# aluo7/ViT-SOM

Hardware: AMD Instinct MI355X
Metric: images/sec/node ViT-SOM 40x40 CIFAR-10 bs512 (training step: fwd+bwd+all-reduce+AdamW) (higher is better)
Workload: dtype f32 (Linear GEMMs on bf16 MFMA: forward from an exact 3xbf16 operand split, six products; weight / input gradients from a 2xbf16 split, three products, rel. error 4e-6)

## Files before the change

vit_som_amd/csrc/bmu_x3.hip:

```cpp
#include "gemm_x6.h"
#include "adamw.h"

#include <type_traits>

namespace vsom {

constexpr float BMU_WINDOW = 2.0e-4f;

struct BmuP {
    const float* X; long ldx; const float* W;
    int B, K, L;
    int ktiles_per_split;
    float* slab; long slab_stride;
    float* xsq; float* wsq;
    unsigned x_bytes, w_bytes;
};

template <int WM, int WN, int WAVES_M, int WAVES_N>
__global__ __launch_bounds__(WAVES_M * WAVES_N * 64) void bmu_x3_kernel(const BmuP g) {
    constexpr int BM = WAVES_M * WM * 32, BN = WAVES_N * WN * 32, NT = WAVES_M * WAVES_N * 64, RPP = NT / 8;
    constexpr int PA = BM * X6_RS, PB = BN * X6_RS;
    __shared__ __attribute__((aligned(16))) char lds[2 * (PA + PB)];
    char* As = lds; char* Bs = lds + 2 * PA;
    const int t = threadIdx.x, lane = t & 63, wave = t >> 6;
// ... 26 lines not shown
    const bool want_x = tn == 0, want_w = tm == 0;
    float ssa[BM / RPP], ssb[BN / RPP];
#pragma unroll
    for (int p = 0; p < BM / RPP; ++p) ssa[p] = 0.f;
#pragma unroll
    for (int p = 0; p < BN / RPP; ++p) ssb[p] = 0.f;

    auto gload = [&](int kt) {
        load_kc_fast<BM, NT>(sa, rsA, oa, kt << 5, g.L, t);
        load_kc_fast<BN, NT>(sb, rsB, ob, kt << 5, g.L, t);
    };
    auto lstore = [&](int) {
#pragma unroll
        for (int p = 0; p < BM / RPP; ++p) {
            const f32x4 v = sa.v[p];
            if (want_x) ssa[p] += (v[0] * v[0] + v[1] * v[1]) + (v[2] * v[2] + v[3] * v[3]);
            uint2 p1, p2;
            x3_split(v, p1, p2);
            char* dst = As + x6_piece_off(p * RPP + (t >> 3), t & 7);
            *reinterpret_cast<uint2*>(dst) = p1;
            *reinterpret_cast<uint2*>(dst + PA) = p2;
        }
#pragma unroll
        for (int p = 0; p < BN / RPP; ++p) {
            const f32x4 v = sb.v[p];
            if (want_w) ssb[p] += (v[0] * v[0] + v[1] * v[1]) + (v[2] * v[2] + v[3] * v[3]);
            uint2 p1, p2;
            x3_split(v, p1, p2);
            char* dst = Bs + x6_piece_off(p * RPP + (t >> 3), t & 7);
            *reinterpret_cast<uint2*>(dst) = p1;
            *reinterpret_cast<uint2*>(dst + PB) = p2;
        }
    };
    auto mfma_tile = [&](int) {
#pragma unroll
        for (int ks = 0; ks < 2; ++ks) {
            bf16x8 a[WM][2], b[WN][2];
#pragma unroll
            for (int i = 0; i < WM; ++i)
#pragma unroll
                for (int pl = 0; pl < 2; ++pl)
                    a[i][pl] = *reinterpret_cast<const bf16x8*>(As + pl * PA + x6_chunk_off(wm0 + i * 32 + r, 2 * ks + h));
#pragma unroll
            for (int j = 0; j < WN; ++j)
#pragma unroll
                for (int pl = 0; pl < 2; ++pl)
                    b[j][pl] = *reinterpret_cast<const bf16x8*>(Bs + pl * PB + x6_chunk_off(wn0 + j * 32 + r, 2 * ks + h));
#pragma unroll
            for (int i = 0; i < WM; ++i)
#pragma unroll
                for (int j = 0; j < WN; ++j) x6_products<2>(acc[i][j], a[i], b[j]);
        }
    };
    X6_KLOOP(1, 2 * (PA + PB), kt_begin, kt_end, gload, lstore, mfma_tile);

    if (want_x) {
#pragma unroll
        for (int p = 0; p < BM / RPP; ++p) {
            float v = ssa[p];
            v += __shfl_xor(v, 1, 64); v += __shfl_xor(v, 2, 64); v += __shfl_xor(v, 4, 64);
            const int m = bm0 + p * RPP + (t >> 3);
            if ((t & 7) == 0 && m < g.B) g.xsq[(long)z * g.B + m] = v;
        }
    }
    if (want_w) {
#pragma unroll
        for (int p = 0; p < BN / RPP; ++p) {
            float v = ssb[p];
            v += __shfl_xor(v, 1, 64); v += __shfl_xor(v, 2, 64); v += __shfl_xor(v, 4, 64);
            const int n = bn0 + p * RPP + (t >> 3);
            if ((t & 7) == 0 && n < g.K) g.wsq[(long)z * g.K + n] = v;
        }
    }
    float* sl = g.slab + (long)z * g.slab_stride;
#pragma unroll
    for (int i = 0; i < WM; ++i)
#pragma unroll
        for (int j = 0; j < WN; ++j) {
            const int n = bn0 + wn0 + j * 32 + r;
            if (n >= g.K) continue;
            const int mb = bm0 + wm0 + i * 32 + 4 * h;
#pragma unroll
            for (int v = 0; v < 16; ++v) {
                const int m = mb + (v & 3) + 8 * (v >> 2);
                if (m < g.B) sl[(long)m * g.K + n] = acc[i][j][v];
            }
        }
}

__global__ __launch_bounds__(256) void bmu_norms_kernel(const float* __restrict__ xsq, const float* __restrict__ wsq, int nz,
                                                        int B, int K, float* __restrict__ inv_nx, float* __restrict__ inv_nw) {
    const int i = blockIdx.x * 256 + threadIdx.x;
    if (i >= B + K) return;
    const bool isx = i < B;
    const float* p = isx ? xsq + i : wsq + (i - B);
    const int n = isx ? B : K;
    float s = 0.f;
    for (int z = 0; z < nz; ++z) s += p[(long)z * n];
    const float inv = 1.0f / fmaxf(sqrtf(s), 1e-12f);
    if (isx) inv_nx[i] = inv; else inv_nw[i - B] = inv;
}

__global__ __launch_bounds__(512) void bmu_norms_wide_kernel(const float* __restrict__ xsq, const float* __restrict__ wsq, int nz,
                                                             int B, int K, float* __restrict__ inv_nx, float* __restrict__ inv_nw) {
    __shared__ float part[8][64];
    const int lane = threadIdx.x & 63, w = threadIdx.x >> 6;
    const int i = blockIdx.x * 64 + lane;
// ... 577 lines not shown
```

vit_som_amd/csrc/gemm_f32.h:

```cpp
#pragma once
#include "common.h"

namespace vsom {

enum Epi : int {
    EPI_NONE = 0,
    EPI_BIAS = 1,
    EPI_BIAS_GELU = 2,
    EPI_BIAS_RES = 3,
    EPI_ROWAXPY = 4,
    EPI_GELU_BWD = 5,
    EPI_SLAB = 6,
    EPI_BIAS_RELU = 7,
    EPI_LN_BWD = 8,
};

struct GemmP {
    const float* A; const float* B; float* C;
    long lda, ldb, ldc;
    int M, N, K;
    int ktiles_per_split;
    int a_seg, a_stride, a_off;
    int c_seg, c_stride, c_off;
    const float* bias;
// ... 81 lines not shown
                v[0] = src[0];
                if (k + 1 < K) v[1] = src[1];
                if (k + 2 < K) v[2] = src[2];
                if (k + 3 < K) v[3] = src[3];
            }
        }
        s.v[p] = v;
    }
}
template <int ROWS>
__device__ __forceinline__ void store_kc(const StageRegs<ROWS>& s, float* lds, int t) {
#pragma unroll
    for (int p = 0; p < ROWS / 32; ++p)
        *reinterpret_cast<f32x4*>(lds + (p * 32 + (t >> 3)) * 36 + ((t & 7) << 2)) = s.v[p];
}
template <int COLS>
__device__ __forceinline__ void load_ks(StageRegs<COLS>& s, const float* __restrict__ base, long ld,
                                        int col0, int ncols, int k0, int K, int vec, int t, int seg,
                                        int stride, int off) {
    constexpr int TPR = COLS / 4;
    constexpr int KPP = 256 / TPR;
#pragma unroll
    for (int p = 0; p < COLS / 32; ++p) {
        const int k = k0 + p * KPP + t / TPR;
        const int col = col0 + ((t % TPR) << 2);
        f32x4 v = {0.f, 0.f, 0.f, 0.f};
        if (k < K && col < ncols) {
            const long row = seg ? (long)(k / seg) * stride + off + (k % seg) : (long)k;
            const float* src = base + row * ld + col;
            if (vec && col + 3 < ncols) {
                v = *reinterpret_cast<const f32x4*>(src);
            } else {
                v[0] = src[0];
                if (col + 1 < ncols) v[1] = src[1];
                if (col + 2 < ncols) v[2] = src[2];
                if (col + 3 < ncols) v[3] = src[3];
            }
        }
        s.v[p] = v;
    }
}
template <int COLS>
__device__ __forceinline__ void store_ks(const StageRegs<COLS>& s, float* lds, int t) {
    constexpr int TPR = COLS / 4;
    constexpr int KPP = 256 / TPR;
#pragma unroll
    for (int p = 0; p < COLS / 32; ++p)
        *reinterpret_cast<f32x4*>(lds + (p * KPP + t / TPR) * (COLS + 4) + ((t % TPR) << 2)) = s.v[p];
}

template <int WM, int WN, int EPI>
__device__ __forceinline__ void gemm_epilogue(const GemmP& g, const f32x16 (&acc)[WM][WN], int m0, int n0, int r, int h, int z) {
    const bool rowmap = (EPI == EPI_BIAS_RES) && g.c_seg != 0;
#pragma unroll
    for (int i = 0; i < WM; ++i) {
#pragma unroll
        for (int j = 0; j < WN; ++j) {
            const int n = n0 + j * 32 + r;
            if (n >= g.N) continue;
            const int mb = m0 + i * 32 + 4 * h;
            float bn = 0.f;
            if constexpr (EPI == EPI_BIAS || EPI == EPI_BIAS_GELU || EPI == EPI_BIAS_RELU || EPI == EPI_BIAS_RES) bn = g.bias ? g.bias[n] : 0.f;
            const bool plain_rows = (m0 + i * 32 + 31 < g.M) && !rowmap &&
                                    !((EPI == EPI_BIAS_RES) && !(g.r_mod >= g.M && g.r_off == 0));
            if (plain_rows) {
                float* d = (EPI == EPI_SLAB) ? g.slab + (long)z * g.slab_stride + (long)mb * g.N + n : g.C + (long)mb * g.ldc + n;
                const long dstep = (EPI == EPI_SLAB) ? (long)g.N : g.ldc;
                const float* rp = nullptr;
                float* d2 = nullptr;
                if constexpr (EPI == EPI_ROWAXPY || EPI == EPI_GELU_BWD || EPI == EPI_BIAS_RES) rp = g.R + (long)mb * g.ldr + n;
                if constexpr (EPI == EPI_BIAS_GELU || EPI == EPI_BIAS_RELU) d2 = g.C2 + (long)mb * g.ldc2 + n;
                const float* rs = nullptr;
                if constexpr (EPI == EPI_ROWAXPY) rs = g.rowscale + mb;
                constexpr bool READS_R = (EPI == EPI_ROWAXPY || EPI == EPI_GELU_BWD || EPI == EPI_BIAS_RES);
                constexpr bool MAY_ACC = (EPI == EPI_NONE || EPI == EPI_ROWAXPY || EPI == EPI_GELU_BWD);
                float rv[16], dv[16];
                if constexpr (READS_R) {
                    const float* q = rp;
#pragma unroll
                    for (int v = 0; v < 16; ++v) { rv[v] = *q; q += (((v & 3) == 3) ? 5 : 1) * g.ldr; }
                }
                float sv[16];
                if constexpr (EPI == EPI_ROWAXPY) {
#pragma unroll
                    for (int v = 0; v < 16; ++v) sv[v] = rs[(v & 3) + 8 * (v >> 2)];
                }
                const bool accum = MAY_ACC && g.accumulate;
                if (accum) {
                    const float* q = d;
#pragma unroll
                    for (int v = 0; v < 16; ++v) { dv[v] = *q; q += (((v & 3) == 3) ? 5 : 1) * dstep; }
                }
#pragma unroll
                for (int v = 0; v < 16; ++v) {
                    const float a = acc[i][j][v];
                    if constexpr (EPI == EPI_SLAB) {
                        *d = a;
                    } else if constexpr (EPI == EPI_NONE) {
                        float val = g.alpha * a;
                        if (accum) val += dv[v];
                        *d = val;
                    } else if constexpr (EPI == EPI_BIAS) {
                        *d = a + bn;
                    } else if constexpr (EPI == EPI_BIAS_GELU) {
                        float act, grad;
                        gelu_erf_both(a + bn, act, grad);
                        *d = grad;
                        *d2 = act;
                    } else if constexpr (EPI == EPI_BIAS_RELU) {
                        const float pre = a + bn;
                        *d = pre > 0.f ? 1.0f : 0.f;
                        *d2 = fmaxf(pre, 0.f);
                    } else if constexpr (EPI == EPI_BIAS_RES) {
                        *d = a + bn + rv[v];
                    } else if constexpr (EPI == EPI_ROWAXPY) {
                        float val = a + sv[v] * rv[v];
                        if (accum) val += dv[v];
                        *d = val;
                    } else if constexpr (EPI == EPI_GELU_BWD) {
                        float val = a * rv[v];
                        if (accum) val += dv[v];
                        *d = val;
                    }
                    const long adv = ((v & 3) == 3) ? 5 : 1;
                    d += adv * dstep;
                    if constexpr (EPI == EPI_BIAS_GELU || EPI == EPI_BIAS_RELU) d2 += adv * g.ldc2;
                }
                continue;
            }
            if constexpr (EPI == EPI_SLAB) {
                float* dst = g.slab + (long)z * g.slab_stride + (long)mb * g.N + n;
#pragma unroll
                for (int v = 0; v < 16; ++v) {
                    const int dm = (v & 3) + 8 * (v >> 2);
                    if (mb + dm < g.M) dst[(long)dm * g.N] = acc[i][j][v];
                }
            } else if (rowmap) {
#pragma unroll
                for (int v = 0; v < 16; ++v) {
                    const int m = mb + (v & 3) + 8 * (v >> 2);
                    if (m >= g.M) continue;
                    const long orow = (long)(m / g.c_seg) * g.c_stride + g.c_off + (m % g.c_seg);
                    const long rr = (long)(m % g.r_mod) + g.r_off;
                    g.C[orow * g.ldc + n] = acc[i][j][v] + bn + g.R[rr * g.ldr + n];
                }
            } else {
                float* dst = g.C + (long)mb * g.ldc + n;
                const float* rsrc = nullptr;
                float* dst2 = nullptr;
                if constexpr (EPI == EPI_ROWAXPY || EPI == EPI_GELU_BWD) rsrc = g.R + (long)mb * g.ldr + n;
                if constexpr (EPI == EPI_BIAS_GELU || EPI == EPI_BIAS_RELU) dst2 = g.C2 + (long)mb * g.ldc2 + n;
                const bool plain_res = (EPI == EPI_BIAS_RES) && g.r_mod >= g.M && g.r_off == 0;
                if constexpr (EPI == EPI_BIAS_RES) rsrc = g.R + (long)mb * g.ldr + n;
#pragma unroll
                for (int v = 0; v < 16; ++v) {
                    const int dm = (v & 3) + 8 * (v >> 2);
                    const int m = mb + dm;
                    if (m >= g.M) continue;
                    const float a = acc[i][j][v];
                    float* d = dst + (long)dm * g.ldc;
                    if constexpr (EPI == EPI_NONE) {
                        float val = g.alpha * a;
                        if (g.accumulate) val += *d;
                        *d = val;
                    } else if constexpr (EPI == EPI_BIAS) {
                        *d = a + bn;
                    } else if constexpr (EPI == EPI_BIAS_GELU) {
                        float act, grad;
                        gelu_erf_both(a + bn, act, grad);
                        *d = grad;
                        dst2[(long)dm * g.ldc2] = act;
                    } else if constexpr (EPI == EPI_BIAS_RELU) {
                        const float pre = a + bn;
// ... 131 lines not shown
                    for (int j = 0; j < WN; ++j)
                        acc[i][j] = __builtin_amdgcn_mfma_f32_32x32x2f32(a[i][s], b[j][s], acc[i][j], 0, 0, 0);
        }
    };
    for (int kt = kt_begin; kt + 1 < kt_end; ++kt) {
        gload(kt + 1);
        __builtin_amdgcn_sched_barrier(0);
        mfma_tile();
        __syncthreads();
        lstore();
        __syncthreads();
    }
    if (kt_begin < kt_end) mfma_tile();

    if constexpr (EPI == EPI_SLAB) {
        if (want_colsum && t < BM && bm0 + t < g.M) g.slab_bias[(long)z * g.slab_bias_stride + bm0 + t] = colsum;
    }
    gemm_epilogue<WM, WN, EPI>(g, acc, bm0 + wm0, bn0 + wn0, r, h, z);
}

enum GemmEngine : int { GEMM_ENGINE_F32 = 0, GEMM_ENGINE_X6 = 1 };
struct GemmPlan {
    int engine;
    int tile_m;
    int planes;
    bool fast;
    int splits;
    int ktiles_per_split;
    int tiles;
    int grid;
};
GemmPlan gemm_plan(bool a_kc, bool b_kc, int epi, int M, int N, int K, bool fast, int mode, int products, int splits);
int gemm_mode();
int launch_gemm(bool a_kc, bool b_kc, int epi, GemmP g, int splits, hipStream_t stream);
int linear_bwd_weight_impl(const float* dY, long lddy, const float* X, long ldx, float* dW, float* db, int M, int N,
                           int K, int a_seg, int a_stride, int a_off, void* ws, size_t ws_bytes,
                           hipStream_t stream);
template <int WAVES, int VEC>
__device__ __forceinline__ void reduce_slabs_body(f32x4 (*sh)[64], int bx, const float* __restrict__ slabs, long stride,
                                                  int nslabs, float* __restrict__ out1, long n1,
                                                  float* __restrict__ out2, long off2, long n2,
                                                  int nb1, int vec) {
    const int lane = threadIdx.x & 63, wave = threadIdx.x >> 6;
    const bool seg2 = bx >= nb1;
    const long col = ((long)(seg2 ? bx - nb1 : bx) * 64 + lane) * VEC;
    const long n = seg2 ? n2 : n1;
    const float* src = slabs + (seg2 ? off2 : 0) + col;
    f32x4 acc[4];
#pragma unroll
    for (int u = 0; u < 4; ++u) acc[u] = f32x4{0.f, 0.f, 0.f, 0.f};
    if (col < n) {
        if (VEC == 4 && vec && col + 3 < n) {
            int s = wave;
            for (; s + 3 * WAVES < nslabs; s += 4 * WAVES) {
#pragma unroll
                for (int u = 0; u < 4; ++u) acc[u] += *reinterpret_cast<const f32x4*>(src + (long)(s + u * WAVES) * stride);
            }
            for (; s < nslabs; s += WAVES) acc[0] += *reinterpret_cast<const f32x4*>(src + (long)s * stride);
        } else if (VEC == 1) {
            int s = wave;
            for (; s + 3 * WAVES < nslabs; s += 4 * WAVES) {
#pragma unroll
                for (int u = 0; u < 4; ++u) acc[u][0] += src[(long)(s + u * WAVES) * stride];
            }
            for (; s < nslabs; s += WAVES) acc[0][0] += src[(long)s * stride];
        } else {
            for (int s = wave; s < nslabs; s += WAVES)
#pragma unroll
                for (int e = 0; e < 4; ++e)
                    if (col + e < n) acc[0][e] += src[(long)s * stride + e];
        }
    }
    sh[wave][lane] = (acc[0] + acc[1]) + (acc[2] + acc[3]);
    __syncthreads();
    if (wave == 0 && col < n) {
        f32x4 t = sh[0][lane];
#pragma unroll
        for (int w = 1; w < WAVES; ++w) t += sh[w][lane];
        float* dst = (seg2 ? out2 : out1) + col;
        if (VEC == 1) {
            dst[0] = t[0];
        } else if (col + 3 < n && (reinterpret_cast<uintptr_t>(dst) & 15u) == 0) {
            *reinterpret_cast<f32x4*>(dst) = t;
        } else {
#pragma unroll
            for (int e = 0; e < 4; ++e)
                if (col + e < n) dst[e] = t[e];
        }
    }
}

int reduce_slabs_internal(const float* slabs, long stride, int nslabs, float* out, long n, hipStream_t stream);
int reduce_slabs2_internal(const float* slabs, long stride, int nslabs, float* out1, long n1, float* out2, long off2,
                           long n2, hipStream_t stream);
int sum_partials(const float* part, int n, float* out, hipStream_t stream);
int choose_splits(int tiles, int ktiles, int max_splits, bool prefer_xcd_multiple = false);
int bmu_splits(int B, int K, int L);
int attn_bwd_threads(int N);
int attn_bwd_plan_now(int N, int hd);
int gemm_grad_products();

}
```

vit_som_amd/csrc/gemm_x6.h:

```cpp
#pragma once
#include "gemm_f32.h"
#include "layernorm_bwd.h"

namespace vsom {

typedef __attribute__((ext_vector_type(8))) __bf16 bf16x8;
typedef unsigned v4u32 __attribute__((ext_vector_type(4)));

__device__ __forceinline__ unsigned x6_bits(float x) { return __builtin_bit_cast(unsigned, x); }
__device__ __forceinline__ float x6_float(unsigned x) { return __builtin_bit_cast(float, x); }

__device__ __forceinline__ void x6_split(f32x4 v, uint2& p1, uint2& p2, uint2& p3) {
    const unsigned HI = 0xffff0000u, SEL = 0x07060302u;
    float r[4], s[4];
#pragma unroll
    for (int e = 0; e < 4; ++e) {
        r[e] = v[e] - x6_float(x6_bits(v[e]) & HI);
        s[e] = r[e] - x6_float(x6_bits(r[e]) & HI);
    }
    p1.x = __builtin_amdgcn_perm(x6_bits(v[1]), x6_bits(v[0]), SEL); p1.y = __builtin_amdgcn_perm(x6_bits(v[3]), x6_bits(v[2]), SEL);
    p2.x = __builtin_amdgcn_perm(x6_bits(r[1]), x6_bits(r[0]), SEL); p2.y = __builtin_amdgcn_perm(x6_bits(r[3]), x6_bits(r[2]), SEL);
    p3.x = __builtin_amdgcn_perm(x6_bits(s[1]), x6_bits(s[0]), SEL); p3.y = __builtin_amdgcn_perm(x6_bits(s[3]), x6_bits(s[2]), SEL);
}

// ... 14 lines not shown

template <int ROWS, int NPL = 3, int NT = 256>
__device__ __forceinline__ void x6_store(const StageRegs<ROWS, NT>& s, char* planes, int t) {
    constexpr int PL = ROWS * X6_RS;
#pragma unroll
    for (int p = 0; p < ROWS * 8 / NT; ++p) {
        uint2 p1, p2, p3;
        if constexpr (NPL == 3) x6_split(s.v[p], p1, p2, p3); else x3_split(s.v[p], p1, p2);
        char* dst = planes + x6_piece_off(p * (NT / 8) + (t >> 3), t & 7);
        *reinterpret_cast<uint2*>(dst) = p1;
        *reinterpret_cast<uint2*>(dst + PL) = p2;
        if constexpr (NPL == 3) *reinterpret_cast<uint2*>(dst + 2 * PL) = p3;
    }
}

struct X6Blk { f32x4 v[4]; };
__device__ __forceinline__ void x6_load_ks(X6Blk& b, __amdgpu_buffer_rsrc_t rsrc, unsigned colbytes, unsigned ld4, int k0,
                                           int K, int kg, int seg, int stride, int off0) {
#pragma unroll
    for (int i = 0; i < 4; ++i) {
        const int k = k0 + 4 * kg + i;
        const unsigned row = seg ? (unsigned)((k / seg) * stride + off0 + (k % seg)) : (unsigned)k;
        b.v[i] = bload4(rsrc, (k < K && colbytes != OOB) ? row * ld4 + colbytes : OOB);
    }
}
template <int NPL = 3>
__device__ __forceinline__ void x6_store_ks(const X6Blk& b, char* planes, int plane_bytes, int mq, int kg) {
#pragma unroll
    for (int e = 0; e < 4; ++e) {
        const f32x4 col = {b.v[0][e], b.v[1][e], b.v[2][e], b.v[3][e]};
        uint2 p1, p2, p3;
        if constexpr (NPL == 3) x6_split(col, p1, p2, p3); else x3_split(col, p1, p2);
        char* dst = planes + x6_piece_off(4 * mq + e, kg);
        *reinterpret_cast<uint2*>(dst) = p1;
        *reinterpret_cast<uint2*>(dst + plane_bytes) = p2;
        if constexpr (NPL == 3) *reinterpret_cast<uint2*>(dst + 2 * plane_bytes) = p3;
    }
}

template <int NPL>
__device__ __forceinline__ void x6_products(f32x16& acc, const bf16x8 (&a)[NPL], const bf16x8 (&b)[NPL]) {
    f32x16 c = acc;
    if constexpr (NPL == 3) {
        c = __builtin_amdgcn_mfma_f32_32x32x16_bf16(a[2], b[0], c, 0, 0, 0);
        c = __builtin_amdgcn_mfma_f32_32x32x16_bf16(a[0], b[2], c, 0, 0, 0);
        c = __builtin_amdgcn_mfma_f32_32x32x16_bf16(a[1], b[1], c, 0, 0, 0);
    }
    c = __builtin_amdgcn_mfma_f32_32x32x16_bf16(a[1], b[0], c, 0, 0, 0);
    c = __builtin_amdgcn_mfma_f32_32x32x16_bf16(a[0], b[1], c, 0, 0, 0);
    c = __builtin_amdgcn_mfma_f32_32x32x16_bf16(a[0], b[0], c, 0, 0, 0);
    acc = c;
}

#define X6_KLOOP(STAGES, ST, kt_begin, kt_end, gload, lstore, mfma_tile)                                                    \
    do {                                                                                                                    \
        static_assert((STAGES) == 1 || (STAGES) == 2, "one or two LDS stages");                                            \
        if constexpr ((STAGES) == 1) {                                                                                      \
            if ((kt_begin) < (kt_end)) {                                                                                    \
                gload(kt_begin);                                                                                            \
                lstore(0);                                                                                                  \
            }                                                                                                               \
            __syncthreads();                                                                                                \
            for (int kt_ = (kt_begin); kt_ + 1 < (kt_end); ++kt_) {                                                         \
                gload(kt_ + 1);                                                                                             \
                __builtin_amdgcn_sched_barrier(0);                                                                          \
                mfma_tile(0);                                                                                               \
                __builtin_amdgcn_sched_barrier(0);                                                                          \
                __syncthreads();                                                                                            \
                lstore(0);                                                                                                  \
                __syncthreads();                                                                                            \
            }                                                                                                               \
            if ((kt_begin) < (kt_end)) mfma_tile(0);                                                                        \
        } else {                                                                                                            \
            if ((kt_begin) < (kt_end)) {                                                                                    \
                gload(kt_begin);                                                                                            \
                lstore(0);                                                                                                  \
                if ((kt_begin) + 1 < (kt_end)) gload((kt_begin) + 1);                                                       \
            }                                                                                                               \
            __syncthreads();                                                                                                \
            int so_ = 0;                                                                                                    \
            for (int kt_ = (kt_begin); kt_ + 1 < (kt_end); ++kt_) {                                                         \
                lstore((ST) - so_);                                                                                         \
                gload(kt_ + 2 < (kt_end) ? kt_ + 2 : kt_ + 1);                                                              \
                __builtin_amdgcn_sched_barrier(0);                                                                          \
                mfma_tile(so_);                                                                                             \
                __builtin_amdgcn_sched_barrier(0);                                                                          \
                __syncthreads();                                                                                            \
                so_ = (ST) - so_;                                                                                           \
            }                                                                                                               \
            if ((kt_begin) < (kt_end)) mfma_tile(so_);                                                                      \
        }                                                                                                                   \
    } while (0)

template <int WN, int WAVES_M, int WAVES_N, int LDS_BYTES>
__device__ __forceinline__ void x6_ln_bwd_epilogue(const GemmP& g, const f32x16 (&acc)[1][WN], char* lds, int bm0, int wm0,
                                                   int wn0, int r, int h, int tile, int t) {
    constexpr int BN = WAVES_N * WN * 32;
    constexpr int cols = BN;
    constexpr int NCH = (BN + 63) / 64;
    constexpr int LROW = BN + 8;
    constexpr int PROWS = WAVES_M * 8;
    constexpr int ITER = PROWS / 16;
    static_assert(PROWS % 16 == 0 && PROWS * LROW * 4 <= LDS_BYTES && 16 * 2 * BN * 4 <= LDS_BYTES, "LN epilogue does not fit");
    float* st = reinterpret_cast<float*>(lds);
    const int sub = t & 15, rg = t >> 4;
    const float inv_n = 1.0f / (float)cols;
    const unsigned rbytes = (unsigned)g.M * cols * 4u;
    const __amdgpu_buffer_rsrc_t rsX = __builtin_amdgcn_make_buffer_rsrc(const_cast<float*>(g.ln_x), 0, (int)rbytes, 0x00020000);
    const __amdgpu_buffer_rsrc_t rsR = __builtin_amdgcn_make_buffer_rsrc(const_cast<float*>(g.ln_resid), 0, (int)rbytes, 0x00020000);
    const __amdgpu_buffer_rsrc_t rsD = __builtin_amdgcn_make_buffer_rsrc(g.C, 0, (int)rbytes, 0x00020000);
    const __amdgpu_buffer_rsrc_t rsM = __builtin_amdgcn_make_buffer_rsrc(const_cast<float*>(g.ln_mean), 0, g.M * 4, 0x00020000);
    const __amdgpu_buffer_rsrc_t rsS = __builtin_amdgcn_make_buffer_rsrc(const_cast<float*>(g.ln_rstd), 0, g.M * 4, 0x00020000);
    const bool has_resid = g.ln_resid != nullptr;
    f32x4 gam[NCH], dg[NCH], db[NCH];
    bool cv[NCH];
#pragma unroll
    for (int j = 0; j < NCH; ++j) {
        cv[j] = 4 * (sub + 16 * j) < cols;
        gam[j] = cv[j] ? reinterpret_cast<const f32x4*>(g.ln_gamma)[sub + 16 * j] : f32x4{0.f, 0.f, 0.f, 0.f};
        dg[j] = f32x4{0.f, 0.f, 0.f, 0.f};
        db[j] = f32x4{0.f, 0.f, 0.f, 0.f};
    }
    const int wr = wm0 >> 5;
#pragma unroll
    for (int q = 0; q < 4; ++q) {
        bool ok[ITER];
        unsigned off[ITER][NCH];
        float mu[ITER], rs[ITER];
        f32x4 xv[ITER][NCH], rr[ITER][NCH];
#pragma unroll
        for (int i = 0; i < ITER; ++i) {
            const int lr = 16 * i + rg;
            const int row = bm0 + (lr >> 3) * 32 + 8 * q + (lr & 7);
            ok[i] = row < g.M;
#pragma unroll
            for (int j = 0; j < NCH; ++j)
                off[i][j] = (ok[i] && cv[j]) ? (unsigned)row * (cols * 4u) + 16u * (sub + 16 * j) : OOB;
            const unsigned roff = ok[i] ? (unsigned)row * 4u : OOB;
            mu[i] = __builtin_bit_cast(float, __builtin_amdgcn_raw_buffer_load_b32(rsM, (int)roff, 0, 0));
            rs[i] = __builtin_bit_cast(float, __builtin_amdgcn_raw_buffer_load_b32(rsS, (int)roff, 0, 0));
#pragma unroll
            for (int j = 0; j < NCH; ++j) {
                xv[i][j] = bload4(rsX, off[i][j]);
                rr[i][j] = has_resid ? bload4(rsR, off[i][j]) : f32x4{0.f, 0.f, 0.f, 0.f};
            }
        }
        __syncthreads();
#pragma unroll
        for (int j = 0; j < WN; ++j)
#pragma unroll
            for (int e = 0; e < 4; ++e) st[(wr * 8 + e + 4 * h) * LROW + wn0 + j * 32 + r] = acc[0][j][4 * q + e];
        __syncthreads();
#pragma unroll
        for (int i = 0; i < ITER; ++i) {
            const int lr = 16 * i + rg;
            f32x4 d[NCH], o[NCH];
#pragma unroll
            for (int j = 0; j < NCH; ++j) {
                d[j] = (cv[j] && ok[i]) ? *reinterpret_cast<const f32x4*>(st + lr * LROW + 4 * (sub + 16 * j)) : f32x4{0.f, 0.f, 0.f, 0.f};
                if (!cv[j]) xv[i][j] = f32x4{mu[i], mu[i], mu[i], mu[i]};
            }
            ln_bwd_row<NCH>(d, xv[i], mu[i], rs[i], gam, inv_n, o, dg, db);
#pragma unroll
            for (int j = 0; j < NCH; ++j) {
                if (has_resid) ln_bwd_add_resid(o[j], rr[i][j]);
                __builtin_amdgcn_raw_buffer_store_b128(__builtin_bit_cast(v4u32, o[j]), rsD, (int)off[i][j], 0, 0);
            }
        }
    }
    __syncthreads();
    float* sh = st;
#pragma unroll
    for (int j = 0; j < NCH; ++j) {
        if (!cv[j]) continue;
        reinterpret_cast<f32x4*>(sh + (rg * 2 + 0) * cols)[sub + 16 * j] = dg[j];
        reinterpret_cast<f32x4*>(sh + (rg * 2 + 1) * cols)[sub + 16 * j] = db[j];
    }
    __syncthreads();
    if (bm0 >= g.M) return;
    for (int c = t; c < 2 * cols; c += 256) {
        float s = 0.f;
#pragma unroll
        for (int q = 0; q < 16; ++q) s += sh[q * 2 * cols + c];
        g.ln_part[(long)tile * 2 * cols + c] = s;
    }
}

template <bool A_KC, bool B_KC, int WM, int WN, int WAVES_M, int WAVES_N, int EPI, int NPL = 3, int NT = 256, int STAGES = 1>
__device__ __forceinline__ void gemm_x6_body(const GemmP& g) {
    constexpr int BM = WAVES_M * WM * 32;
    constexpr int BN = WAVES_N * WN * 32;
    constexpr int PA = BM * X6_RS, PB = BN * X6_RS;
    constexpr int ST = NPL * (PA + PB);
    static_assert(NT == WAVES_M * WAVES_N * 64 && (NT == 256 || (A_KC && B_KC)), "thread count");
    constexpr int RG = NT / 256;
    constexpr int LN_NEED = EPI == EPI_LN_BWD ? 16 * 2 * BN * 4 : 0;
    constexpr int LDS_BYTES = STAGES * ST > RG * LN_NEED ? STAGES * ST : RG * LN_NEED;
    __shared__ __attribute__((aligned(16))) char lds[LDS_BYTES];
    char* As = lds;
    char* Bs = lds + NPL * PA;

    const int t = threadIdx.x;
    const int lane = t & 63, wave = t >> 6;
    const int r = lane & 31, h = lane >> 5;
    const int wm0 = (wave / WAVES_N) * (WM * 32);
    const int wn0 = (wave % WAVES_N) * (WN * 32);

    const int tiles_n = (g.N + BN - 1) / BN;
    const int tiles_m = (g.M + BM - 1) / BM;
    const int ntiles = tiles_m * tiles_n;
    const int lid = xcd_remap(blockIdx.x, gridDim.x);
    const int z = lid / ntiles;
    const int rem = lid - z * ntiles;
    const int tm = g.n_major ? rem % tiles_m : rem / tiles_n;
    const int tn = g.n_major ? rem / tiles_m : rem % tiles_n;
    const int bm0 = tm * BM;
    const int bn0 = tn * BN;

    const int ktiles = (g.K + 31) >> 5;
    const int kt_begin = z * g.ktiles_per_split;
    int kt_end = kt_begin + g.ktiles_per_split;
    if (kt_end > ktiles) kt_end = ktiles;

    f32x16 acc[WM][WN];
#pragma unroll
    for (int i = 0; i < WM; ++i)
#pragma unroll
        for (int j = 0; j < WN; ++j)
#pragma unroll
            for (int v = 0; v < 16; ++v) acc[i][j][v] = 0.f;

    const __amdgpu_buffer_rsrc_t rsA = __builtin_amdgcn_make_buffer_rsrc(const_cast<float*>(g.A), 0, (int)g.a_bytes, 0x00020000);
// ... 3 lines not shown
    OffKC<A_KC ? BM : 32, NT> oa; OffKC<B_KC ? BN : 32, NT> ob;
    constexpr int TA = 2 * BM, TB0 = 256 - 2 * BN;
    static_assert((A_KC || TA <= 256) && (B_KC || TB0 >= 0), "tile too large for the k-strided task map");
    const bool has_a = !A_KC && t < TA, has_b = !B_KC && t >= TB0;
    const int kga = t & 7, mqa = t >> 3, kgb = (t - TB0) & 7, mqb = (t - TB0) >> 3;
    X6Blk ba, bb;
    unsigned cola = OOB, colb = OOB;
    float cs[4] = {0.f, 0.f, 0.f, 0.f};
    const bool want_colsum = (EPI == EPI_SLAB) && !A_KC && g.slab_bias != nullptr && bn0 == 0;
    if constexpr (A_KC) init_kc<BM, NT>(oa, g.lda, bm0, g.M, t);
    else if (has_a && bm0 + 4 * mqa < g.M) cola = (unsigned)(bm0 + 4 * mqa) << 2;
    if constexpr (B_KC) init_kc<BN, NT>(ob, g.ldb, bn0, g.N, t);
    else if (has_b && bn0 + 4 * mqb < g.N) colb = (unsigned)(bn0 + 4 * mqb) << 2;
    auto gload = [&](int kt) {
        if constexpr (A_KC) load_kc_fast<BM, NT>(sa, rsA, oa, kt << 5, g.K, t);
        else if (has_a) x6_load_ks(ba, rsA, cola, (unsigned)g.lda << 2, kt << 5, g.K, kga, g.a_seg, g.a_stride, g.a_off);
        if constexpr (B_KC) load_kc_fast<BN, NT>(sb, rsB, ob, kt << 5, g.K, t);
        else if (has_b) x6_load_ks(bb, rsB, colb, (unsigned)g.ldb << 2, kt << 5, g.K, kgb, 0, 0, 0);
    };
    auto lstore = [&](int so) {
        if constexpr (A_KC) {
            x6_store<BM, NPL, NT>(sa, As + so, t);
        } else if (has_a) {
            if (want_colsum) {
#pragma unroll
                for (int e = 0; e < 4; ++e) cs[e] += (ba.v[0][e] + ba.v[1][e]) + (ba.v[2][e] + ba.v[3][e]);
            }
            x6_store_ks<NPL>(ba, As + so, PA, mqa, kga);
        }
        if constexpr (B_KC) x6_store<BN, NPL, NT>(sb, Bs + so, t);
        else if (has_b) x6_store_ks<NPL>(bb, Bs + so, PB, mqb, kgb);
    };

    auto mfma_tile = [&](int so) {
#pragma unroll
        for (int ks = 0; ks < 2; ++ks) {
            bf16x8 a[WM][NPL], b[WN][NPL];
#pragma unroll
            for (int i = 0; i < WM; ++i)
#pragma unroll
                for (int pl = 0; pl < NPL; ++pl)
                    a[i][pl] = *reinterpret_cast<const bf16x8*>(As + so + pl * PA + x6_chunk_off(wm0 + i * 32 + r, 2 * ks + h));
#pragma unroll
            for (int j = 0; j < WN; ++j)
#pragma unroll
                for (int pl = 0; pl < NPL; ++pl)
                    b[j][pl] = *reinterpret_cast<const bf16x8*>(Bs + so + pl * PB + x6_chunk_off(wn0 + j * 32 + r, 2 * ks + h));
#pragma unroll
            for (int i = 0; i < WM; ++i)
#pragma unroll
                for (int j = 0; j < WN; ++j) x6_products<NPL>(acc[i][j], a[i], b[j]);
        }
    };
    X6_KLOOP(STAGES, ST, kt_begin, kt_end, gload, lstore, mfma_tile);
    if constexpr (EPI == EPI_SLAB && !A_KC) {
        if (want_colsum && has_a) {
#pragma unroll
            for (int e = 0; e < 4; ++e) {
                float v = cs[e];
                v += __shfl_xor(v, 1, 64); v += __shfl_xor(v, 2, 64); v += __shfl_xor(v, 4, 64);
                const int m = bm0 + 4 * mqa + e;
                if (kga == 0 && m < g.M) g.slab_bias[(long)z * g.slab_bias_stride + m] = v;
            }
        }
    }
    if constexpr (EPI == EPI_LN_BWD) {
        static_assert(A_KC && B_KC && WM == 1 && WAVES_M % RG == 0, "EPI_LN_BWD: NT GEMM, one accumulator row per wave");
        constexpr int GM = WAVES_M / RG * 32, RGS = (LDS_BYTES / RG) & ~15;
        const int gi = t >> 8;
        x6_ln_bwd_epilogue<WN, WAVES_M / RG, WAVES_N, RGS>(g, acc, lds + gi * RGS, bm0 + gi * GM, wm0 - gi * GM, wn0, r, h,
                                                           tm * RG + gi, t & 255);
    } else {
        gemm_epilogue<WM, WN, EPI>(g, acc, bm0 + wm0, bn0 + wn0, r, h, z);
    }
}

template <bool A_KC, bool B_KC, int WM, int WN, int WAVES_M, int WAVES_N, int EPI, int NPL = 3>
__global__ __launch_bounds__(256) void gemm_x6_kernel(const GemmP g) {
    gemm_x6_body<A_KC, B_KC, WM, WN, WAVES_M, WAVES_N, EPI, NPL>(g);
}

template <int WN, int WAVES_M, int WAVES_N, int NPL>
__global__ __launch_bounds__(256, 2) void gemm_x6_ln_kernel(const GemmP g) {
    gemm_x6_body<true, true, 1, WN, WAVES_M, WAVES_N, EPI_LN_BWD, NPL>(g);
}

template <int WN, int WAVES_M, int WAVES_N, int NPL>
__global__ __launch_bounds__(WAVES_M * WAVES_N * 64) void gemm_x6_ln_wide_kernel(const GemmP g) {
    gemm_x6_body<true, true, 1, WN, WAVES_M, WAVES_N, EPI_LN_BWD, NPL, WAVES_M * WAVES_N * 64, 2>(g);
}

}
```

vit_som_amd/csrc/gemm_x6_tn.h:

```cpp
#pragma once
#include "gemm_x6.h"

namespace vsom {

typedef __attribute__((ext_vector_type(4))) short s16x4;
typedef __attribute__((ext_vector_type(8))) short s16x8;

struct TnP {
    const float* dY; const float* X;
    long ldy, ldx;
    int T, NO, KI;
    int ktiles_per_split;
    int a_seg, a_stride, a_off;
    float* slab; long slab_stride;
    float* slab_bias; long slab_bias_stride;
    unsigned a_bytes, b_bytes;
};

constexpr int tn_stride(int C) { return ((C * 2 + 63) / 128) * 128 + 64; }

__device__ __forceinline__ s16x4 tn_trread(const char* p) {
    return __builtin_amdgcn_ds_read_tr16_b64_v4i16((__attribute__((address_space(3))) s16x4*)p);
}

// ... 60 lines not shown
    };
    auto lstore = [&](int so) {
#pragma unroll
        for (int i = 0; i < FA; ++i) {
            if (la[i] < 0) continue;
            if (want_colsum) cs[i] += sa[i];
            uint2 p1, p2, p3;
            if constexpr (NPL == 3) x6_split(sa[i], p1, p2, p3); else x3_split(sa[i], p1, p2);
            *reinterpret_cast<uint2*>(As + so + la[i]) = p1;
            *reinterpret_cast<uint2*>(As + so + PA + la[i]) = p2;
            if constexpr (NPL == 3) *reinterpret_cast<uint2*>(As + so + 2 * PA + la[i]) = p3;
        }
#pragma unroll
        for (int i = 0; i < FB; ++i) {
            if (lb[i] < 0) continue;
            uint2 p1, p2, p3;
            if constexpr (NPL == 3) x6_split(sb[i], p1, p2, p3); else x3_split(sb[i], p1, p2);
            *reinterpret_cast<uint2*>(Bs + so + lb[i]) = p1;
            *reinterpret_cast<uint2*>(Bs + so + PB + lb[i]) = p2;
            if constexpr (NPL == 3) *reinterpret_cast<uint2*>(Bs + so + 2 * PB + lb[i]) = p3;
        }
    };
    const int G = lane >> 4, q = (lane >> 2) & 3, pp = lane & 3;
    const int trow = 8 * (G >> 1) + q, tcol = 16 * (G & 1) + 4 * pp;
    int fa[WM], fbo[WN];
#pragma unroll
    for (int i = 0; i < WM; ++i) fa[i] = trow * SA + (wm0 + i * 32 + tcol) * 2;
#pragma unroll
    for (int j = 0; j < WN; ++j) fbo[j] = trow * SB + (wn0 + j * 32 + tcol) * 2;
    auto frag = [&](const char* base, int off, int stride, int ks) -> bf16x8 {
        const s16x4 lo = tn_trread(base + off + (ks * 16) * stride);
        const s16x4 hi = tn_trread(base + off + (ks * 16 + 4) * stride);
        const s16x8 v = {lo[0], lo[1], lo[2], lo[3], hi[0], hi[1], hi[2], hi[3]};
        return __builtin_bit_cast(bf16x8, v);
    };
    auto mfma_tile = [&](int so) {
#pragma unroll
        for (int ks = 0; ks < 2; ++ks) {
            bf16x8 a[WM][NPL], b[WN][NPL];
#pragma unroll
            for (int i = 0; i < WM; ++i)
#pragma unroll
                for (int pl = 0; pl < NPL; ++pl) a[i][pl] = frag(As + so + pl * PA, fa[i], SA, ks);
#pragma unroll
            for (int j = 0; j < WN; ++j)
#pragma unroll
                for (int pl = 0; pl < NPL; ++pl) b[j][pl] = frag(Bs + so + pl * PB, fbo[j], SB, ks);
#pragma unroll
            for (int i = 0; i < WM; ++i)
#pragma unroll
                for (int j = 0; j < WN; ++j) x6_products<NPL>(acc[i][j], a[i], b[j]);
        }
    };
    X6_KLOOP(STAGES, ST, kt_begin, kt_end, gload, lstore, mfma_tile);

    if (want_colsum) {
        __syncthreads();
        f32x4* park = reinterpret_cast<f32x4*>(lds);
#pragma unroll
        for (int i = 0; i < FA; ++i) park[i * NT + t] = cs[i];
        __syncthreads();
        if (t < BM) {
            const int c4 = t >> 2, e = t & 3;
            float s = 0.f;
#pragma unroll 8
            for (int row = 0; row < 32; ++row) s += reinterpret_cast<const float*>(&park[row * (BM / 4) + c4])[e];
            g.slab_bias[(long)z * g.slab_bias_stride + bm0 + t] = s;
        }
    }
    const int r = lane & 31, h = lane >> 5;
    float* sl = g.slab + (long)z * g.slab_stride;
#pragma unroll
    for (int i = 0; i < WM; ++i)
#pragma unroll
        for (int j = 0; j < WN; ++j) {
            float* d = sl + (long)(bm0 + wm0 + i * 32 + 4 * h) * g.KI + bn0 + wn0 + j * 32 + r;
#pragma unroll
            for (int v = 0; v < 16; ++v) {
                *d = acc[i][j][v];
                d += (((v & 3) == 3) ? 5 : 1) * (long)g.KI;
            }
        }
}

}
```

Measured before the change: 59190.

## Prefetch epilogue loads ahead of last MFMA tile and across LN-bwd passes

Adds a before_last hook to the K-loop macro so the LayerNorm-backward epilogue issues its x, mean, rstd and residual loads before the final MFMA tile. Restructures the LN-bwd epilogue to prefetch the next pass's loads while computing the current one. Also hoists residual and rowscale loads in the generic GEMM epilogue ahead of the store loop, and adds a 12-deep unrolled slab reduction loop. These changes hide global-memory latency behind compute, at the cost of higher register pressure and possible occupancy loss.

```diff
diff --git a/vit_som_amd/csrc/bmu_x3.hip b/vit_som_amd/csrc/bmu_x3.hip
--- a/vit_som_amd/csrc/bmu_x3.hip
+++ b/vit_som_amd/csrc/bmu_x3.hip
@@ -102,7 +102,7 @@
                 for (int j = 0; j < WN; ++j) x6_products<2>(acc[i][j], a[i], b[j]);
         }
     };
-    X6_KLOOP(1, 2 * (PA + PB), kt_begin, kt_end, gload, lstore, mfma_tile);
+    X6_KLOOP(1, 2 * (PA + PB), kt_begin, kt_end, gload, lstore, mfma_tile, );
 
     if (want_x) {
 #pragma unroll
diff --git a/vit_som_amd/csrc/gemm_f32.h b/vit_som_amd/csrc/gemm_f32.h
--- a/vit_som_amd/csrc/gemm_f32.h
+++ b/vit_som_amd/csrc/gemm_f32.h
@@ -157,6 +157,29 @@
 template <int WM, int WN, int EPI>
 __device__ __forceinline__ void gemm_epilogue(const GemmP& g, const f32x16 (&acc)[WM][WN], int m0, int n0, int r, int h, int z) {
     const bool rowmap = (EPI == EPI_BIAS_RES) && g.c_seg != 0;
+    auto plain = [&](int i) {
+        return (m0 + i * 32 + 31 < g.M) && !rowmap && !((EPI == EPI_BIAS_RES) && !(g.r_mod >= g.M && g.r_off == 0));
+    };
+    constexpr bool READS_R = (EPI == EPI_ROWAXPY || EPI == EPI_GELU_BWD || EPI == EPI_BIAS_RES);
+    float rv[WM][WN][16], sv[WM][WN][16];
+    if constexpr (READS_R) {
+#pragma unroll
+        for (int i = 0; i < WM; ++i) {
+#pragma unroll
+            for (int j = 0; j < WN; ++j) {
+                const int n = n0 + j * 32 + r;
+                if (n >= g.N || !plain(i)) continue;
+                const int mb = m0 + i * 32 + 4 * h;
+                const float* q = g.R + (long)mb * g.ldr + n;
+#pragma unroll
+                for (int v = 0; v < 16; ++v) { rv[i][j][v] = *q; q += (((v & 3) == 3) ? 5 : 1) * g.ldr; }
+                if constexpr (EPI == EPI_ROWAXPY) {
+#pragma unroll
+                    for (int v = 0; v < 16; ++v) sv[i][j][v] = g.rowscale[mb + (v & 3) + 8 * (v >> 2)];
+                }
+            }
+        }
+    }
 #pragma unroll
     for (int i = 0; i < WM; ++i) {
 #pragma unroll
@@ -166,30 +189,13 @@
             const int mb = m0 + i * 32 + 4 * h;
             float bn = 0.f;
             if constexpr (EPI == EPI_BIAS || EPI == EPI_BIAS_GELU || EPI == EPI_BIAS_RELU || EPI == EPI_BIAS_RES) bn = g.bias ? g.bias[n] : 0.f;
-            const bool plain_rows = (m0 + i * 32 + 31 < g.M) && !rowmap &&
-                                    !((EPI == EPI_BIAS_RES) && !(g.r_mod >= g.M && g.r_off == 0));
-            if (plain_rows) {
+            if (plain(i)) {
                 float* d = (EPI == EPI_SLAB) ? g.slab + (long)z * g.slab_stride + (long)mb * g.N + n : g.C + (long)mb * g.ldc + n;
                 const long dstep = (EPI == EPI_SLAB) ? (long)g.N : g.ldc;
-                const float* rp = nullptr;
                 float* d2 = nullptr;
-                if constexpr (EPI == EPI_ROWAXPY || EPI == EPI_GELU_BWD || EPI == EPI_BIAS_RES) rp = g.R + (long)mb * g.ldr + n;
                 if constexpr (EPI == EPI_BIAS_GELU || EPI == EPI_BIAS_RELU) d2 = g.C2 + (long)mb * g.ldc2 + n;
-                const float* rs = nullptr;
-                if constexpr (EPI == EPI_ROWAXPY) rs = g.rowscale + mb;
-                constexpr bool READS_R = (EPI == EPI_ROWAXPY || EPI == EPI_GELU_BWD || EPI == EPI_BIAS_RES);
                 constexpr bool MAY_ACC = (EPI == EPI_NONE || EPI == EPI_ROWAXPY || EPI == EPI_GELU_BWD);
-                float rv[16], dv[16];
-                if constexpr (READS_R) {
-                    const float* q = rp;
-#pragma unroll
-                    for (int v = 0; v < 16; ++v) { rv[v] = *q; q += (((v & 3) == 3) ? 5 : 1) * g.ldr; }
-                }
-                float sv[16];
-                if constexpr (EPI == EPI_ROWAXPY) {
-#pragma unroll
-                    for (int v = 0; v < 16; ++v) sv[v] = rs[(v & 3) + 8 * (v >> 2)];
-                }
+                float dv[16];
                 const bool accum = MAY_ACC && g.accumulate;
                 if (accum) {
                     const float* q = d;
@@ -217,13 +223,13 @@
                         *d = pre > 0.f ? 1.0f : 0.f;
                         *d2 = fmaxf(pre, 0.f);
                     } else if constexpr (EPI == EPI_BIAS_RES) {
-                        *d = a + bn + rv[v];
+                        *d = a + bn + rv[i][j][v];
                     } else if constexpr (EPI == EPI_ROWAXPY) {
-                        float val = a + sv[v] * rv[v];
+                        float val = a + sv[i][j][v] * rv[i][j][v];
                         if (accum) val += dv[v];
                         *d = val;
                     } else if constexpr (EPI == EPI_GELU_BWD) {
-                        float val = a * rv[v];
+                        float val = a * rv[i][j][v];
                         if (accum) val += dv[v];
                         *d = val;
                     }
@@ -461,6 +467,18 @@
     if (col < n) {
         if (VEC == 4 && vec && col + 3 < n) {
             int s = wave;
+            for (; s + 11 * WAVES < nslabs; s += 12 * WAVES) {
+                f32x4 v[3][4];
+#pragma unroll
+                for (int i = 0; i < 3; ++i)
+#pragma unroll
+                    for (int u = 0; u < 4; ++u) v[i][u] = *reinterpret_cast<const f32x4*>(src + (long)(s + (4 * i + u) * WAVES) * stride);
+                __builtin_amdgcn_sched_barrier(0);
+#pragma unroll
+                for (int i = 0; i < 3; ++i)
+#pragma unroll
+                    for (int u = 0; u < 4; ++u) acc[u] += v[i][u];
+            }
             for (; s + 3 * WAVES < nslabs; s += 4 * WAVES) {
 #pragma unroll
                 for (int u = 0; u < 4; ++u) acc[u] += *reinterpret_cast<const f32x4*>(src + (long)(s + u * WAVES) * stride);
diff --git a/vit_som_amd/csrc/gemm_x6.h b/vit_som_amd/csrc/gemm_x6.h
--- a/vit_som_amd/csrc/gemm_x6.h
+++ b/vit_som_amd/csrc/gemm_x6.h
@@ -90,7 +90,7 @@
     acc = c;
 }
 
-#define X6_KLOOP(STAGES, ST, kt_begin, kt_end, gload, lstore, mfma_tile)                                                    \
+#define X6_KLOOP(STAGES, ST, kt_begin, kt_end, gload, lstore, mfma_tile, before_last)                                       \
     do {                                                                                                                    \
         static_assert((STAGES) == 1 || (STAGES) == 2, "one or two LDS stages");                                            \
         if constexpr ((STAGES) == 1) {                                                                                      \
@@ -108,6 +108,7 @@
                 lstore(0);                                                                                                  \
                 __syncthreads();                                                                                            \
             }                                                                                                               \
+            before_last;                                                                                                    \
             if ((kt_begin) < (kt_end)) mfma_tile(0);                                                                        \
         } else {                                                                                                            \
             if ((kt_begin) < (kt_end)) {                                                                                    \
@@ -126,30 +127,78 @@
                 __syncthreads();                                                                                            \
                 so_ = (ST) - so_;                                                                                           \
             }                                                                                                               \
+            before_last;                                                                                                    \
             if ((kt_begin) < (kt_end)) mfma_tile(so_);                                                                      \
         }                                                                                                                   \
     } while (0)
 
-template <int WN, int WAVES_M, int WAVES_N, int LDS_BYTES>
-__device__ __forceinline__ void x6_ln_bwd_epilogue(const GemmP& g, const f32x16 (&acc)[1][WN], char* lds, int bm0, int wm0,
-                                                   int wn0, int r, int h, int tile, int t) {
-    constexpr int BN = WAVES_N * WN * 32;
-    constexpr int cols = BN;
-    constexpr int NCH = (BN + 63) / 64;
+template <int WN, int WAVES_M, int WAVES_N>
+struct LnBwdLoads {
+    static constexpr int BN = WAVES_N * WN * 32;
+    static constexpr int cols = BN;
+    static constexpr int NCH = (BN + 63) / 64;
+    static constexpr int PROWS = WAVES_M * 8;
+    static constexpr int ITER = PROWS / 16;
+    struct Pass {
+        unsigned base[ITER];
+        float mu[ITER], rs[ITER];
+        f32x4 xv[ITER][NCH];
+    };
+    typedef f32x4 Resid[ITER][NCH];
+    __device__ __forceinline__ unsigned off(unsigned base, int j) const {
+        return (base != OOB && 4 * (sub + 16 * j) < cols) ? base + 256u * j : OOB;
+    }
+    __amdgpu_buffer_rsrc_t rsX, rsR, rsM, rsS;
+    bool has_resid;
+    int M, bm0, sub, rg;
+    __device__ __forceinline__ void init(const GemmP& g, int bm0_, int t) {
+        const unsigned rbytes = (unsigned)g.M * cols * 4u;
+        rsX = __builtin_amdgcn_make_buffer_rsrc(const_cast<float*>(g.ln_x), 0, (int)rbytes, 0x00020000);
+        rsR = __builtin_amdgcn_make_buffer_rsrc(const_cast<float*>(g.ln_resid), 0, (int)rbytes, 0x00020000);
+        rsM = __builtin_amdgcn_make_buffer_rsrc(const_cast<float*>(g.ln_mean), 0, g.M * 4, 0x00020000);
+        rsS = __builtin_amdgcn_make_buffer_rsrc(const_cast<float*>(g.ln_rstd), 0, g.M * 4, 0x00020000);
+        has_resid = g.ln_resid != nullptr;
+        M = g.M; bm0 = bm0_; sub = t & 15; rg = t >> 4;
+    }
+    __device__ __forceinline__ void load(int q, Pass& p) const {
+#pragma unroll
+        for (int i = 0; i < ITER; ++i) {
+            const int lr = 16 * i + rg;
+            const int row = bm0 + (lr >> 3) * 32 + 8 * q + (lr & 7);
+            p.base[i] = row < M ? (unsigned)row * (cols * 4u) + 16u * sub : OOB;
+            const unsigned roff = row < M ? (unsigned)row * 4u : OOB;
+            p.mu[i] = __builtin_bit_cast(float, __builtin_amdgcn_raw_buffer_load_b32(rsM, (int)roff, 0, 0));
+            p.rs[i] = __builtin_bit_cast(float, __builtin_amdgcn_raw_buffer_load_b32(rsS, (int)roff, 0, 0));
+#pragma unroll
+            for (int j = 0; j < NCH; ++j) p.xv[i][j] = bload4(rsX, off(p.base[i], j));
+        }
+        __builtin_amdgcn_sched_barrier(0);
+    }
+    __device__ __forceinline__ void load_resid(const Pass& p, Resid& rr) const {
+        __builtin_amdgcn_sched_barrier(0);
+#pragma unroll
+        for (int i = 0; i < ITER; ++i)
+#pragma unroll
+            for (int j = 0; j < NCH; ++j) rr[i][j] = has_resid ? bload4(rsR, off(p.base[i], j)) : f32x4{0.f, 0.f, 0.f, 0.f};
+        __builtin_amdgcn_sched_barrier(0);
+    }
+};
+
+template <int WN, int WAVES_M, int WAVES_N, int LDS_BYTES, bool AHEAD>
+__device__ __forceinline__ void x6_ln_bwd_epilogue(const GemmP& g, const f32x16 (&acc)[1][WN], char* lds,
+                                                   const LnBwdLoads<WN, WAVES_M, WAVES_N>& ld,
+                                                   typename LnBwdLoads<WN, WAVES_M, WAVES_N>::Pass& pre0,
+                                                   typename LnBwdLoads<WN, WAVES_M, WAVES_N>::Resid& rr, int wm0, int wn0,
+                                                   int r, int h, int tile, int t) {
+    typedef LnBwdLoads<WN, WAVES_M, WAVES_N> L;
+    constexpr int BN = L::BN, cols = L::cols, NCH = L::NCH, PROWS = L::PROWS, ITER = L::ITER;
     constexpr int LROW = BN + 8;
-    constexpr int PROWS = WAVES_M * 8;
-    constexpr int ITER = PROWS / 16;
     static_assert(PROWS % 16 == 0 && PROWS * LROW * 4 <= LDS_BYTES && 16 * 2 * BN * 4 <= LDS_BYTES, "LN epilogue does not fit");
     float* st = reinterpret_cast<float*>(lds);
     const int sub = t & 15, rg = t >> 4;
     const float inv_n = 1.0f / (float)cols;
-    const unsigned rbytes = (unsigned)g.M * cols * 4u;
-    const __amdgpu_buffer_rsrc_t rsX = __builtin_amdgcn_make_buffer_rsrc(const_cast<float*>(g.ln_x), 0, (int)rbytes, 0x00020000);
-    const __amdgpu_buffer_rsrc_t rsR = __builtin_amdgcn_make_buffer_rsrc(const_cast<float*>(g.ln_resid), 0, (int)rbytes, 0x00020000);
-    const __amdgpu_buffer_rsrc_t rsD = __builtin_amdgcn_make_buffer_rsrc(g.C, 0, (int)rbytes, 0x00020000);
-    const __amdgpu_buffer_rsrc_t rsM = __builtin_amdgcn_make_buffer_rsrc(const_cast<float*>(g.ln_mean), 0, g.M * 4, 0x00020000);
-    const __amdgpu_buffer_rsrc_t rsS = __builtin_amdgcn_make_buffer_rsrc(const_cast<float*>(g.ln_rstd), 0, g.M * 4, 0x00020000);
-    const bool has_resid = g.ln_resid != nullptr;
+    const __amdgpu_buffer_rsrc_t rsD = __builtin_amdgcn_make_buffer_rsrc(g.C, 0, (int)((unsigned)g.M * cols * 4u), 0x00020000);
+    const bool has_resid = ld.has_resid;
     f32x4 gam[NCH], dg[NCH], db[NCH];
     bool cv[NCH];
 #pragma unroll
@@ -160,52 +209,47 @@
         db[j] = f32x4{0.f, 0.f, 0.f, 0.f};
     }
     const int wr = wm0 >> 5;
-#pragma unroll
-    for (int q = 0; q < 4; ++q) {
-        bool ok[ITER];
-        unsigned off[ITER][NCH];
-        float mu[ITER], rs[ITER];
-        f32x4 xv[ITER][NCH], rr[ITER][NCH];
+    typename L::Pass pre1;
+    auto pass = [&](int q, typename L::Pass& in, typename L::Pass& nx) {
+        if constexpr (AHEAD) {
+            if (q + 1 < 4) ld.load(q + 1, nx);
+        } else if (q > 0) {
+            ld.load(q, in);
+            ld.load_resid(in, rr);
+        }
+        __syncthreads();
+#pragma unroll
+        for (int j = 0; j < WN; ++j)
+#pragma unroll
+            for (int e = 0; e < 4; ++e) st[(wr * 8 + e + 4 * h) * LROW + wn0 + j * 32 + r] = acc[0][j][4 * q + e];
+        __syncthreads();
+        f32x4 o[ITER][NCH];
 #pragma unroll
         for (int i = 0; i < ITER; ++i) {
             const int lr = 16 * i + rg;
-            const int row = bm0 + (lr >> 3) * 32 + 8 * q + (lr & 7);
-            ok[i] = row < g.M;
+            const float mu = in.mu[i], rs = in.rs[i];
+            f32x4 d[NCH], xv[NCH];
+#pragma unroll
+            for (int j = 0; j < NCH; ++j) {
+                d[j] = (cv[j] && in.base[i] != OOB) ? *reinterpret_cast<const f32x4*>(st + lr * LROW + 4 * (sub + 16 * j)) : f32x4{0.f, 0.f, 0.f, 0.f};
+                xv[j] = cv[j] ? in.xv[i][j] : f32x4{mu, mu, mu, mu};
+            }
+            ln_bwd_row<NCH>(d, xv, mu, rs, gam, inv_n, o[i], dg, db);
 #pragma unroll
             for (int j = 0; j < NCH; ++j)
-                off[i][j] = (ok[i] && cv[j]) ? (unsigned)row * (cols * 4u) + 16u * (sub + 16 * j) : OOB;
-            const unsigned roff = ok[i] ? (unsigned)row * 4u : OOB;
-            mu[i] = __builtin_bit_cast(float, __builtin_amdgcn_raw_buffer_load_b32(rsM, (int)roff, 0, 0));
-            rs[i] = __builtin_bit_cast(float, __builtin_amdgcn_raw_buffer_load_b32(rsS, (int)roff, 0, 0));
-#pragma unroll
-            for (int j = 0; j < NCH; ++j) {
-                xv[i][j] = bload4(rsX, off[i][j]);
-                rr[i][j] = has_resid ? bload4(rsR, off[i][j]) : f32x4{0.f, 0.f, 0.f, 0.f};
-            }
-        }
-        __syncthreads();
-#pragma unroll
-        for (int j = 0; j < WN; ++j)
-#pragma unroll
-            for (int e = 0; e < 4; ++e) st[(wr * 8 + e + 4 * h) * LROW + wn0 + j * 32 + r] = acc[0][j][4 * q + e];
-        __syncthreads();
-#pragma unroll
-        for (int i = 0; i < ITER; ++i) {
-            const int lr = 16 * i + rg;
-            f32x4 d[NCH], o[NCH];
-#pragma unroll
-            for (int j = 0; j < NCH; ++j) {
-                d[j] = (cv[j] && ok[i]) ? *reinterpret_cast<const f32x4*>(st + lr * LROW + 4 * (sub + 16 * j)) : f32x4{0.f, 0.f, 0.f, 0.f};
-                if (!cv[j]) xv[i][j] = f32x4{mu[i], mu[i], mu[i], mu[i]};
-            }
-            ln_bwd_row<NCH>(d, xv[i], mu[i], rs[i], gam, inv_n, o, dg, db);
-#pragma unroll
-            for (int j = 0; j < NCH; ++j) {
-                if (has_resid) ln_bwd_add_resid(o[j], rr[i][j]);
-                __builtin_amdgcn_raw_buffer_store_b128(__builtin_bit_cast(v4u32, o[j]), rsD, (int)off[i][j], 0, 0);
-            }
-        }
-    }
+                if (has_resid) ln_bwd_add_resid(o[i][j], rr[i][j]);
+        }
+        if (AHEAD && q + 1 < 4) ld.load_resid(nx, rr);
+#pragma unroll
+        for (int i = 0; i < ITER; ++i)
+#pragma unroll
+            for (int j = 0; j < NCH; ++j)
+                __builtin_amdgcn_raw_buffer_store_b128(__builtin_bit_cast(v4u32, o[i][j]), rsD, (int)ld.off(in.base[i], j), 0, 0);
+    };
+    pass(0, pre0, pre1);
+    pass(1, AHEAD ? pre1 : pre0, pre0);
+    pass(2, pre0, pre1);
+    pass(3, AHEAD ? pre1 : pre0, pre0);
     __syncthreads();
     float* sh = st;
 #pragma unroll
@@ -215,7 +259,7 @@
         reinterpret_cast<f32x4*>(sh + (rg * 2 + 1) * cols)[sub + 16 * j] = db[j];
     }
     __syncthreads();
-    if (bm0 >= g.M) return;
+    if (ld.bm0 >= g.M) return;
     for (int c = t; c < 2 * cols; c += 256) {
         float s = 0.f;
 #pragma unroll
@@ -325,7 +369,19 @@
                 for (int j = 0; j < WN; ++j) x6_products<NPL>(acc[i][j], a[i], b[j]);
         }
     };
-    X6_KLOOP(STAGES, ST, kt_begin, kt_end, gload, lstore, mfma_tile);
+    constexpr int GM = WAVES_M / RG * 32;
+    typedef LnBwdLoads<WN, EPI == EPI_LN_BWD ? WAVES_M / RG : 2, WAVES_N> LnLoads;
+    LnLoads ln_ld;
+    typename LnLoads::Pass ln_pre;
+    typename LnLoads::Resid ln_rr;
+    auto before_last = [&]() {
+        if constexpr (EPI == EPI_LN_BWD) {
+            ln_ld.init(g, bm0 + (t >> 8) * GM, t & 255);
+            ln_ld.load(0, ln_pre);
+            ln_ld.load_resid(ln_pre, ln_rr);
+        }
+    };
+    X6_KLOOP(STAGES, ST, kt_begin, kt_end, gload, lstore, mfma_tile, before_last());
     if constexpr (EPI == EPI_SLAB && !A_KC) {
         if (want_colsum && has_a) {
 #pragma unroll
@@ -339,9 +395,10 @@
     }
     if constexpr (EPI == EPI_LN_BWD) {
         static_assert(A_KC && B_KC && WM == 1 && WAVES_M % RG == 0, "EPI_LN_BWD: NT GEMM, one accumulator row per wave");
-        constexpr int GM = WAVES_M / RG * 32, RGS = (LDS_BYTES / RG) & ~15;
+        constexpr int RGS = (LDS_BYTES / RG) & ~15;
         const int gi = t >> 8;
-        x6_ln_bwd_epilogue<WN, WAVES_M / RG, WAVES_N, RGS>(g, acc, lds + gi * RGS, bm0 + gi * GM, wm0 - gi * GM, wn0, r, h,
+        x6_ln_bwd_epilogue<WN, WAVES_M / RG, WAVES_N, RGS, RG != 1 || BM != 64>(g, acc, lds + gi * RGS, ln_ld, ln_pre, ln_rr, wm0 - gi * GM, wn0,
+                                                           r, h,
                                                            tm * RG + gi, t & 255);
     } else {
         gemm_epilogue<WM, WN, EPI>(g, acc, bm0 + wm0, bn0 + wn0, r, h, z);
diff --git a/vit_som_amd/csrc/gemm_x6_tn.h b/vit_som_amd/csrc/gemm_x6_tn.h
--- a/vit_som_amd/csrc/gemm_x6_tn.h
+++ b/vit_som_amd/csrc/gemm_x6_tn.h
@@ -136,7 +136,7 @@
                 for (int j = 0; j < WN; ++j) x6_products<NPL>(acc[i][j], a[i], b[j]);
         }
     };
-    X6_KLOOP(STAGES, ST, kt_begin, kt_end, gload, lstore, mfma_tile);
+    X6_KLOOP(STAGES, ST, kt_begin, kt_end, gload, lstore, mfma_tile, );
 
     if (want_colsum) {
         __syncthreads();
```

Result: no change. 58710 (-0.8%).
